# amzn/pecos

Hardware: AMD Instinct MI355X
Metric: XLinear queries/sec @ beam=10 top-k=10; P@1 vs reference; 1/2/4/8 GPU (higher is better)
Workload: dtype f32; 1 GPU; amazon-670k synthetic x1.0: N=490000 D=135000 L=670091 tree=[2, 32, 512, 8192, 670091] nnz/row=75.4 beam=10 topk=10 pp=l3-hinge bias=1.0; parallelism=query-shard x1

## Files before the change

pecos_amd/csrc/xrl_abi.cpp:

```cpp
#include "../../include/xrl_abi.h"

#include <algorithm>
#include <cfloat>
#include <chrono>
#include <cmath>
#include <cstdio>
#include <cstring>
#include <functional>
#include <condition_variable>
#include <memory>
#include <mutex>
#include <atomic>
#include <thread>
#include <unordered_map>

#include "xrl_predict.h"
#include "xrl_tfidf.h"

using namespace xrl;

namespace {
thread_local std::string g_err;
thread_local bool g_has_err = false;
thread_local int g_device = 0;
// ... 1265 lines not shown
    uint32_t n = 0;
    guarded([&] {
        Model& m = *as_model(model);
        resolve_profile(m);
        n = (uint32_t)m.profile.size();
        for (uint32_t i = 0; i < n && i < cap && out; ++i) {
            std::memset(&out[i], 0, sizeof(out[i]));
            std::strncpy(out[i].name, m.profile[i].name.c_str(), sizeof(out[i].name) - 1);
            out[i].layer = m.profile[i].layer; out[i].launches = m.profile[i].launches;
            out[i].ms = m.profile[i].ms;
        }
    });
    return n;
}

uint32_t xrl_debug_split_chunk(const uint64_t* cum, uint32_t n, uint64_t limit) {
    uint32_t v = 0;
    guarded([&] { if (!cum) fail("null cum"); v = split_chunk(cum, n, limit); });
    return v;
}

uint64_t xrl_debug_layout_rows(const uint32_t* rptr, uint32_t nrows, int align, uint32_t* ext_out) {
    uint64_t v = 0;
    guarded([&] { if (!rptr) fail("null rptr"); v = layout_tile_rows(rptr, nrows, align != 0, ext_out); });
    return v;
}

static void set_option_one(Model& m, const char* key, int64_t value) {
    if (!std::strcmp(key, "k1_group")) m.k1_group = (int)value;
    else if (!std::strcmp(key, "max_batch_rows")) m.max_batch_rows = value;
    else if (!std::strcmp(key, "sort_min_tiles")) m.sort_min_tiles = (int)value;
    else if (!std::strcmp(key, "sort_rest")) m.sort_rest = (int)value;
    else if (!std::strcmp(key, "prune_mid")) m.prune_mid = (int)value;
    else if (!std::strcmp(key, "tile_rows")) m.tile_rows = (int)value;
    else if (!std::strcmp(key, "k2_big_min_k")) m.k2_big_min_k = (int)value;
    else if (!std::strcmp(key, "qsort")) m.qsort = (int)value;
    else if (!std::strcmp(key, "qsort_min_parents")) m.qsort_min_parents = (int)value;
    else if (!std::strcmp(key, "qsort_min_rows")) m.qsort_min_rows = (int)value;
    else if (!std::strcmp(key, "presence")) m.presence = (int)value;
    else if (!std::strcmp(key, "adaptive")) { m.adaptive = (int)value; for (auto& u : m.fb_unstaged) u = 0; for (auto& u : m.fb_probing) u = 0; }
    else if (!std::strcmp(key, "host_pipeline")) m.host_pipeline = (int)value;
    else if (!std::strcmp(key, "host_batch_mb")) m.host_batch_mb = (int)value;
    else if (!std::strcmp(key, "sort_rest_min")) m.sort_rest_min = (int)value;
    else if (!std::strcmp(key, "reserve_rows")) {
        if (value < 0 || value > 0x7FFFFFFF) fail("reserve_rows: expected 0 .. 2^31-1");
        std::lock_guard<std::mutex> g(m.mu);
        use_device(m.device);
        if (!m.ws) m.ws = std::make_unique<Workspace>();
        reserve_outputs(m, (uint32_t)value, effective_topk(m, 0));
    }
    else if (!std::strcmp(key, "host_register")) m.host_register = (int)value;
    else if (!std::strcmp(key, "k1q_fuse")) m.k1q_fuse = (int)value;
    else if (!std::strcmp(key, "k1g_first")) m.k1g_first = (int)value;
    else if (!std::strcmp(key, "k1g_min_items")) m.k1g_min_items = (int)value;
    else if (!std::strcmp(key, "dense_layers")) m.dense_layers = (int)value;
    else if (!std::strcmp(key, "overlap_min_rows")) m.overlap_min_rows = (int)value;
    else if (!std::strcmp(key, "prune")) m.prune = (int)value;
    else if (!std::strcmp(key, "k1g_variant")) m.k1g_variant = (int)value;
    else if (!std::strcmp(key, "k1_wpb")) m.k1_wpb = (int)value;
    else if (!std::strcmp(key, "k1_lds_pad")) m.k1_lds_pad = (int)value;
    else if (!std::strcmp(key, "k1_ablate")) m.k1_ablate = (int)value;
    else fail(std::string("unknown option ") + key);
}


int xrl_set_option(void* model, const char* key, int64_t value) {
    int rc = -1;
    guarded([&] {
        Model& m = *as_model(model);
        if (!key) fail("null key");
        if (!std::strcmp(key, "devices")) {
            if (value < 1 || value > 64) fail("devices: expected 1..64");
            if (m.src_kind < 0 && value > 1) fail("devices: only models loaded from a folder can be replicated");
            std::lock_guard<std::mutex> g(m.mu);
            int ndev = 0;
            XRL_HIP(hipGetDeviceCount(&ndev));
            m.replicas.clear();
            for (int64_t i = 1; i < value; ++i) {
                const int dev = (m.device + (int)i) % std::max(1, ndev);
                use_device(dev);
                std::unique_ptr<Model> r = m.src_kind == 0 ? load_model_from_disk(m.src_path, m.weight_matrix_type) : load_mmap_model_from_disk(m.src_path);
                r->device = dev;
                r->k1_group = m.k1_group; r->max_batch_rows = m.max_batch_rows; r->sort_min_tiles = m.sort_min_tiles; r->sort_rest = m.sort_rest; r->sort_rest_min = m.sort_rest_min; r->prune_mid = m.prune_mid; r->tile_rows = m.tile_rows; r->k2_big_min_k = m.k2_big_min_k; r->qsort = m.qsort; r->qsort_min_parents = m.qsort_min_parents; r->qsort_min_rows = m.qsort_min_rows; r->presence = m.presence; r->adaptive = m.adaptive; r->host_pipeline = m.host_pipeline; r->host_batch_mb = m.host_batch_mb; r->host_register = m.host_register;
                r->k1q_fuse = m.k1q_fuse; r->k1g_min_items = m.k1g_min_items; r->k1g_first = m.k1g_first; r->dense_layers = m.dense_layers;
                r->overlap_min_rows = m.overlap_min_rows; r->prune = m.prune;
                r->k1g_variant = m.k1g_variant; r->k1_wpb = m.k1_wpb; r->k1_lds_pad = m.k1_lds_pad; r->k1_ablate = m.k1_ablate;
                m.replicas.push_back(std::move(r));
            }
            use_device(m.device);
        } else {
            set_option_one(m, key, value);
            for (auto& r : m.replicas) set_option_one(*r, key, value);
        }
        rc = 0;
    });
    return rc;
}

void xrl_debug_k1_phases(unsigned long long* out8, int reset) { guarded([&] { k1_phase_read(out8, reset != 0); }); }

uint32_t xrl_layer_info(void* model, uint32_t layer, uint64_t* out, uint32_t cap) {
    uint32_t n = 0;
    guarded([&] {
        Model& m = *as_model(model);
        if (layer >= m.layers.size()) fail("xrl_layer_info: layer out of range");
        const Layer& L = *m.layers[layer];
        const uint64_t rec[12] = {
            (uint64_t)(L.dev.bucket ? 1 : (L.dev.bitmap64 ? 2 : 0)), L.bk_levels, (uint64_t)(L.dev.wd ? 1 : 0), 1ull << L.dev.d_gp_log2,
            L.dev.d_ld, L.n_tiles, L.nnz, L.dense_bytes, L.w_rows, L.n_children, L.max_tile_cols, L.device_bytes};
        n = 12;
        for (uint32_t i = 0; i < n && i < cap && out; ++i) out[i] = rec[i];
    });
    return n;
}

uint64_t xrl_model_device_bytes(void* model) {
// ... 271 lines not shown
```

pecos_amd/csrc/xrl_device.h:

```cpp
#pragma once
#include <hip/hip_runtime.h>

#include <cfloat>
#include <cmath>

#include "xrl_model.h"

namespace xrl {

__device__ __forceinline__ void wave_sync_lds() {
    __builtin_amdgcn_fence(__ATOMIC_SEQ_CST, "wavefront");
    __builtin_amdgcn_wave_barrier();
}

__device__ __forceinline__ bool prune_guard_ok(uint32_t xmax_bits, uint32_t n_feat, float wmax) {
    if (xmax_bits >= 0x7F800000u) return false;
    const float b = fmaxf(__uint_as_float(xmax_bits), 1.0f) * wmax * (float)(n_feat + 2u);
    return b < 1.0e37f;
}

__device__ __forceinline__ float ref_expf(float x) { return (float)exp((double)x); }

__device__ __forceinline__ double hinge_pow4(float zf, int p) {
    const double z = (double)zf;
// ... 95 lines not shown
template <int NS>
__device__ __forceinline__ uint32_t wave_topk_extract(uint32_t (&kx)[NS], const uint32_t (&sbits)[NS], const uint32_t (&payload)[NS],
                                                      uint32_t k, int lane, uint32_t& o_rank, uint32_t& o_sbits, uint32_t& o_payload) {
    uint32_t osb = 0, opl = 0, i = 0;
    for (; i < k; ++i) {
        uint32_t m = kx[0];
#pragma unroll
        for (int r = 1; r < NS; ++r) m = max(m, kx[r]);
        const uint32_t mx = wave_max_u32(m);
        if (mx == 0u) break;
        bool found = false;
#pragma unroll
        for (int r = 0; r < NS; ++r) {
            if (!found) {
                const unsigned long long b = __ballot(kx[r] == mx);
                if (b != 0ull) {
                    const int wl = __builtin_ctzll(b);
                    const int sb = __builtin_amdgcn_readlane((int)sbits[r], wl), pl = __builtin_amdgcn_readlane((int)payload[r], wl);
                    const bool dst = (uint32_t)lane == i;
                    osb = dst ? (uint32_t)sb : osb;
                    opl = dst ? (uint32_t)pl : opl;
                    kx[r] = lane == wl ? 0u : kx[r];
                    found = true;
                }
            }
        }
    }
    o_rank = (uint32_t)lane; o_sbits = osb; o_payload = opl;
    return i;
}
constexpr uint32_t kTopkExtractMaxK = 20;

template <int NS>
__device__ __forceinline__ uint32_t wave_topk(uint32_t (&key)[NS], const uint32_t (&sbits)[NS], const uint32_t (&payload)[NS],
                                              uint32_t k, uint2* sc, int lane, uint32_t& o_rank, uint32_t& o_sbits, uint32_t& o_payload) {
    if (k <= kTopkExtractMaxK) return wave_topk_extract<NS>(key, sbits, payload, k, lane, o_rank, o_sbits, o_payload);
    o_rank = 0; o_sbits = 0; o_payload = 0;
    const uint32_t n_valid = wave_count_ge<NS>(key, 1u);
    const uint32_t kk = min(k, n_valid);
    if (kk == 0) return 0;
    uint32_t lo = 1u, hi = 0xFFFFFFFFu;
    bool exact = false;
    if (NS >= 4) {
        uint32_t m[1] = {key[0]};
#pragma unroll
        for (int r = 1; r < NS; ++r) m[0] = max(m[0], key[r]);
        uint32_t mx = m[0];
#pragma unroll
        for (int d = 1; d < 64; d <<= 1) mx = max(mx, (uint32_t)__shfl_xor((int)mx, d, 64));
        hi = __builtin_amdgcn_readfirstlane(mx);
        bool e1;
        lo = wave_bisect_kth<1>(m, kk, 0u, hi, e1);
        if (lo == 0u) lo = 1u;
    }
    const uint32_t T = wave_bisect_kth<NS>(key, kk, lo, hi, exact);
    uint32_t need_eq = 0;
    if (!exact) need_eq = kk - (T == 0xFFFFFFFFu ? 0u : wave_count_ge<NS>(key, T + 1u));
    uint32_t base = 0, eq_seen = 0;
#pragma unroll
    for (int r = 0; r < NS; ++r) {
        const bool above = exact ? key[r] >= T : key[r] > T;
        const bool eq = !exact && key[r] == T;
        const unsigned long long meq = __ballot(eq);
        const bool sel = above || (eq && eq_seen + lanes_below(meq) < need_eq);
        const unsigned long long msel = __ballot(sel);
        if (sel) sc[base + lanes_below(msel)] = make_uint2(sbits[r], payload[r]);
// ... 17 lines not shown
```

pecos_amd/csrc/xrl_k1t.hip:

```cpp
#include <hip/hip_runtime.h>

#include <cfloat>
#include <cmath>

#include "xrl_device.h"
#include "xrl_kernels.h"
#include "xrl_items.h"

namespace xrl {

#define XRL_LAUNCH_CHECK() XRL_HIP(hipGetLastError())

namespace {

__device__ __forceinline__ uint32_t xcd_remap_t(uint32_t b, uint32_t nb) {
    const uint32_t xcd = b & 7u, q = nb >> 3, r = nb & 7u;
    const uint32_t base = (xcd < r) ? xcd * (q + 1u) : r * (q + 1u) + (xcd - r) * q;
    return base + (b >> 3);
}

struct K1TArgs {
    LayerDev L;
    QueriesDev X;
    const ItemDesc* items;
    const uint32_t* n_items;
    float* cand;
    uint64_t n_slots;
    int pp_kind, pp_p, first_layer, bias_first;
    uint32_t n_vblocks;
    uint32_t* fb_out;
    uint32_t wt_bytes;
};

template <int NR> struct RowVec;
template <> struct RowVec<1> { float v[1]; };
template <> struct alignas(8) RowVec<2> { float v[2]; };
template <> struct RowVec<3> { float v[3]; };
template <> struct alignas(16) RowVec<4> { float v[4]; };

typedef uint32_t u32x2 __attribute__((ext_vector_type(2)));
typedef uint32_t u32x3 __attribute__((ext_vector_type(3)));
typedef uint32_t u32x4 __attribute__((ext_vector_type(4)));
template <int NR> __device__ __forceinline__ RowVec<NR> row_load_buf(__amdgpu_buffer_rsrc_t rs, uint32_t voff);
template <> __device__ __forceinline__ RowVec<1> row_load_buf<1>(__amdgpu_buffer_rsrc_t rs, uint32_t voff) { return __builtin_bit_cast(RowVec<1>, __builtin_amdgcn_raw_buffer_load_b32(rs, (int)voff, 0, 0)); }
template <> __device__ __forceinline__ RowVec<2> row_load_buf<2>(__amdgpu_buffer_rsrc_t rs, uint32_t voff) { return __builtin_bit_cast(RowVec<2>, __builtin_amdgcn_raw_buffer_load_b64(rs, (int)voff, 0, 0)); }
template <> __device__ __forceinline__ RowVec<3> row_load_buf<3>(__amdgpu_buffer_rsrc_t rs, uint32_t voff) {
    const auto t = __builtin_amdgcn_raw_buffer_load_b96(rs, (int)voff, 0, 0);
    RowVec<3> r; r.v[0] = __uint_as_float(t[0]); r.v[1] = __uint_as_float(t[1]); r.v[2] = __uint_as_float(t[2]); return r;
}
template <> __device__ __forceinline__ RowVec<4> row_load_buf<4>(__amdgpu_buffer_rsrc_t rs, uint32_t voff) { return __builtin_bit_cast(RowVec<4>, __builtin_amdgcn_raw_buffer_load_b128(rs, (int)voff, 0, 0)); }

template <int G, int NR, int PPC, int LK, bool BUF>
__global__ void __launch_bounds__(256) __attribute__((amdgpu_waves_per_eu(5, 8))) k1t_kernel(K1TArgs a) {
    constexpr int W = 64 / G, H = 64, U = (G >= 16) ? 64 / G : 8, UNR = 8, STRIDE = G * NR;
    __shared__ uint2 hq_all[4 * W * (H + UNR)];
    const uint32_t wave = threadIdx.x >> 6;
    const uint32_t vblock = blockIdx.x * 4u + wave;
    if (vblock >= a.n_vblocks) return;
    const int lane = threadIdx.x & 63;
    const int grp = lane / G, lig = lane % G;
    uint2* __restrict__ my_hq = hq_all + ((size_t)wave * W + grp) * (H + UNR);

    ItemDesc it = make_item(0u, kNoTile, 0u, 0.f, 0, 0u);
    if (a.n_items) {
        const uint32_t n = *a.n_items, nb = (n + W - 1) / W;
        if (a.fb_out && vblock == 0 && lane == 0) *a.fb_out = n;
        if (vblock >= nb) return;
        { const uint64_t slot = (uint64_t)xcd_remap_t(vblock, nb) * W + grp; if (slot < n) it = a.items[slot]; }
    } else {
        const uint64_t slot = (uint64_t)vblock * W + grp;
        if (slot < a.n_slots) it = a.items[slot];
    }
    const bool active = it.tile != kNoTile;
    TileDesc td{};
    uint64_t xe = 0, cur = 0, wbase = 0;
    if (active) {
        td = a.L.tiles[it.tile];
        wbase = a.L.wt_base[it.tile];
        cur = it.x_begin; xe = it.x_begin + it.x_len;
    }
    const char* __restrict__ wrow = reinterpret_cast<const char*>(a.L.wt + (BUF ? 0ull : wbase) + (uint32_t)(NR * lig));
    const uint32_t tbase = BUF ? (uint32_t)(wbase * 4ull) : 0u;
    const uint32_t lane_off = (uint32_t)(NR * lig * 4);
    const __amdgpu_buffer_rsrc_t wrs = __builtin_amdgcn_make_buffer_rsrc(const_cast<float*>(a.L.wt), 0, (int)(BUF ? a.wt_bytes : 0u), 0x00020000);
    const uint32_t pad_off = tbase + td.nrows * (uint32_t)(STRIDE * 4);
    float acc[NR];
    {
        const float* __restrict__ bp = a.L.bias_prod + td.col_begin;
#pragma unroll
        for (int k = 0; k < NR; ++k) {
            const uint32_t c = (uint32_t)(NR * lig + k);
            acc[k] = (a.bias_first && a.L.has_bias && c < td.ncols) ? bp[c] : 0.0f;
        }
    }
    const uint32_t* __restrict__ xi = a.X.col_idx;
    const float* __restrict__ xv = a.X.val;
    const BmWord* __restrict__ bm = a.L.bitmap + (LK != 0 ? 0ull : (uint64_t)(active ? it.tile : 0u) * a.L.nwords);
    const BmWord64* __restrict__ bm64 = a.L.bitmap64 + (LK != 2 ? 0ull : (uint64_t)(active ? it.tile : 0u) * a.L.nwords64);
    const unsigned long long below = (1ull << lig) - 1ull;
    const uint64_t xlast = xe > cur ? xe - 1 : 0;
    uint32_t nh = 0;
    bool nonfin = false;

    auto drain = [&](auto exact_tag) {
        constexpr bool EX = decltype(exact_tag)::value;
        wave_sync_lds();
// ... 60 lines not shown
#pragma unroll
                for (int u = 0; u < U; ++u) {
                    const bool inr = f[u] != 0xFFFFFFFFu;
                    const BmWord64 wi = bm64[inr ? (f[u] >> 6) : 0u];
                    const uint32_t b = f[u] & 63u;
                    const unsigned long long bits = ((unsigned long long)wi.hi << 32) | wi.lo;
                    hit[u] = inr && ((bits >> b) & 1ull);
                    off[u] = tbase + (wi.rank + (uint32_t)__popcll(bits & ((1ull << b) - 1ull))) * (uint32_t)(STRIDE * 4);
                }
            }
            uint32_t done = skip;
            bool stopped = false;
#pragma unroll
            for (int u = 0; u < U; ++u) {
                const unsigned long long m = __ballot(hit[u]);
                const unsigned long long gm = (G == 64) ? m : ((m >> (grp * G)) & ((1ull << G) - 1ull));
                const uint32_t cnt = (uint32_t)__popcll(gm);
                if ((uint32_t)u >= done && !stopped) {
                    if (nh + cnt <= (uint32_t)H) {
                        if (hit[u]) my_hq[nh + (uint32_t)__popcll(gm & below)] = make_uint2(__float_as_uint(v[u]), off[u]);
                        nh += cnt; done = u + 1;
                    } else {
                        stopped = true;
                    }
                }
            }
            if (done == (uint32_t)U) { if (cur < xe) cur += (uint64_t)U * G; skip = 0; }
            else { skip = done; overflow = true; }
        }
        if (__any(overflow)) drain_any();
    }
    drain_any();

    if (!active) return;
    float* __restrict__ out = a.cand + it.out_off;
    const float* __restrict__ bp = a.L.bias_prod + td.col_begin;
    const bool add_bias = a.L.has_bias != 0 && !a.bias_first;
#pragma unroll
    for (int k = 0; k < NR; ++k) {
        const uint32_t c = (uint32_t)(NR * lig + k);
        if (c < td.ncols) {
            float s = acc[k];
            if (add_bias) s = __fadd_rn(s, bp[c]);
            float v = pp_transform<PPC>(a.pp_kind, a.pp_p, s);
            if (!a.first_layer) v = pp_combine(a.pp_kind, v, it.pscore);
            out[c] = v;
        }
    }
}

__global__ void __launch_bounds__(256)
tile_rows_kernel(const TileDesc* __restrict__ tiles, const uint32_t* __restrict__ row_ext, const Entry* __restrict__ entries,
                 const uint64_t* __restrict__ wt_base, uint32_t stride, uint32_t* __restrict__ wt) {
    const TileDesc td = tiles[blockIdx.x];
    uint32_t* __restrict__ dst = wt + wt_base[blockIdx.x];
    const uint32_t* __restrict__ ext = row_ext + td.rowptr_base;
    const Entry* __restrict__ ent = entries + td.ent_base;
    const uint32_t sub = threadIdx.x >> 5, l = threadIdx.x & 31u;
    for (uint32_t r = sub; r < td.nrows; r += 8u) {
        const uint32_t e = ext[r], start = e & 0x1FFFFFFu, len = (e >> 25) + 1u;
        for (uint32_t i = l; i < len; i += 32u) {
            const Entry x = ent[start + i];
            const uint32_t b = __float_as_uint(x.val);
            dst[(uint64_t)r * stride + x.col] = b == kMissing ? 0u : b;
        }
    }
}

}

void k1t_shape(uint32_t max_tile_cols, int& g, int& nr) {
    g = max_tile_cols <= 8 ? 8 : max_tile_cols <= 16 ? 16 : 32;
    nr = (int)((max_tile_cols + (uint32_t)g - 1) / (uint32_t)g);
    if (nr < 1) nr = 1;
}

void launch_tile_rows(const LayerDev& L, uint64_t total_floats, uint32_t* wt, hipStream_t s) {
    XRL_HIP(hipMemsetD32Async(reinterpret_cast<hipDeviceptr_t>(wt), (int)kMissing, total_floats, s));
    if (L.n_tiles) {
        hipLaunchKernelGGL(tile_rows_kernel, dim3(L.n_tiles), dim3(256), 0, s, L.tiles, L.row_ext, L.entries, L.wt_base, L.wt_stride, wt);
        XRL_LAUNCH_CHECK();
    }
}

bool k1t_serves(const LayerDev& L, const QueriesDev& X) { return L.wt != nullptr && !X.dense && (L.bitmap || L.bitmap64) && !L.bucket; }

void launch_k1t(const LayerDev& L, const LayerPlan& P, const QueriesDev& X, const void* items, const uint32_t* n_items, float* cand, hipStream_t s) {
    if (P.nrows == 0) return;
    K1TArgs a;
    a.L = L; a.X = X; a.items = static_cast<const ItemDesc*>(items); a.n_items = n_items; a.cand = cand;
    a.n_slots = (uint64_t)P.nrows * P.beam_in * L.max_tiles_per_parent;
    a.pp_kind = P.pp.kind; a.pp_p = P.pp.p; a.first_layer = P.first_layer; a.bias_first = P.bias_first;
    a.fb_out = (n_items && P.fb_host && P.layer >= 0 && P.layer < 16) ? P.fb_host + 32 + P.layer : nullptr;
    int g, nr;
    k1t_shape(L.max_tile_cols, g, nr);
    if ((uint32_t)(g * nr) != L.wt_stride || nr > 4) fail("k1t: the layer's tile rows were laid out for another shape");
    const uint64_t vblocks = (a.n_slots + (uint64_t)(64 / g) - 1) / (uint64_t)(64 / g);
    if (vblocks > 0x7FFFFFFFull) fail("k1t: grid too large; lower max_batch_rows");
    a.n_vblocks = (uint32_t)vblocks;
    const dim3 grid((uint32_t)((vblocks + 3) / 4)), block(256);
    const int ppc = pp_class(P.pp);
    const int lk = L.bitmap64 ? 2 : 0;
    const bool buf = L.wt_bytes != 0 && L.wt_bytes < 0xFFFFFF00ull;
    a.wt_bytes = buf ? (uint32_t)L.wt_bytes : 0u;
#define XRL_K1T_B(GG, NN, BB) do { \
        if (ppc) { if (lk) hipLaunchKernelGGL((k1t_kernel<GG, NN, 1, 2, BB>), grid, block, 0, s, a); else hipLaunchKernelGGL((k1t_kernel<GG, NN, 1, 0, BB>), grid, block, 0, s, a); } \
        else     { if (lk) hipLaunchKernelGGL((k1t_kernel<GG, NN, 0, 2, BB>), grid, block, 0, s, a); else hipLaunchKernelGGL((k1t_kernel<GG, NN, 0, 0, BB>), grid, block, 0, s, a); } } while (0)
#define XRL_K1T(GG, NN) do { if (buf) XRL_K1T_B(GG, NN, true); else XRL_K1T_B(GG, NN, false); } while (0)
    if (g == 8) XRL_K1T(8, 1);
    else if (g == 16) XRL_K1T(16, 1);
    else if (nr == 1) XRL_K1T(32, 1);
    else if (nr == 2) XRL_K1T(32, 2);
    else if (nr == 3) XRL_K1T(32, 3);
    else XRL_K1T(32, 4);
#undef XRL_K1T
#undef XRL_K1T_B
    XRL_LAUNCH_CHECK();
}

}
```

pecos_amd/csrc/xrl_kernels.h:

```cpp
#pragma once
#include "xrl_model.h"

namespace xrl {

struct QueriesDev {
    const uint64_t* row_ptr;
    const uint32_t* col_idx;
    const float* val;
    uint32_t rows, cols;
    int dense;
    uint64_t nnz;
};

struct BeamDev {
    uint32_t* idx;
    float* val;
    uint32_t* cnt;
    uint32_t stride;
};

struct K1Tune { int wpb = 1, lds_pad = 0, ablate = 0, k1g_variant = 0, pres_mode = 1, tile_rows = 1, k2_big_min_k = 0; };

struct LayerPlan {
    uint32_t row0, nrows;
// ... 31 lines not shown
void launch_k2_topk(const LayerDev& L, const LayerPlan& P, BeamDev prev, const uint32_t* cand_off,
                    const uint32_t* ncand, const float* cand, uint32_t* out_idx, float* out_val,
                    uint32_t* out_cnt, uint32_t out_stride, hipStream_t s,
                    uint32_t rank_limit = 0 , uint32_t limited_cands = 0 ,
                    uint32_t* done = nullptr , const uint32_t* skip_done = nullptr ,
                    const uint32_t* xok = nullptr );
constexpr int kStatsPerLayer = 8;
void launch_stats(const LayerDev& L, const LayerPlan& P, const QueriesDev& X, BeamDev prev, const uint32_t* ncand, const void* items,
                  double* out8, hipStream_t s, uint64_t item_slots = 0 );
void launch_k3_inner_products(const uint64_t* x_ptr, const uint32_t* x_idx, const float* x_val, int x_dense,
                              const uint64_t* w_ptr, const uint32_t* w_idx, const float* w_val, int w_dense,
                              uint32_t dim, uint64_t len, const uint32_t* rows, const uint32_t* cols,
                              float* out, hipStream_t s);

unsigned long long* k1_phase_buffer();
void k1_phase_read(unsigned long long out[8], bool reset);
void launch_k4_selected(const uint64_t* col_ptr, const uint32_t* row_idx, const float* val, uint32_t w_rows, float bias,
                        const QueriesDev& X, const uint32_t* pair_q, const uint32_t* node, const uint32_t* ppos,
                        const uint64_t* prev_off, const float* prev_val, float* out_val, uint64_t n_pairs,
                        const PostProc& pp, int first_layer, hipStream_t s);
uint32_t k1g_cols(const LayerDev& L);
void launch_k1g(const LayerDev& L, const LayerPlan& P, const QueriesDev& X, const void* items_sorted, const uint32_t* start,
                uint32_t* blk_start, const uint32_t* x_ok, float* cand, hipStream_t s);
void launch_xguard(const QueriesDev& X, uint32_t row0, uint32_t nrows, float wmax, uint32_t* ok, hipStream_t s);
void launch_k1c_csc(const LayerDev& L, const uint64_t* col_ptr, const uint32_t* row_idx, const float* val, const LayerPlan& P,
                    const QueriesDev& X, BeamDev prev, const uint32_t* cand_off, const uint32_t* ncand, float* cand, hipStream_t s);
void launch_concat_csr(const uint64_t* in_ptr, const uint32_t* in_idx, const float* in_val, const float* emb, uint32_t rows,
                       uint32_t sparse_cols, uint32_t dense_cols, int normalize_emb, uint64_t* out_ptr, uint32_t* out_idx, float* out_val, hipStream_t s);
void launch_tfidf_weight(const uint64_t* row_ptr, const uint32_t* col_idx, const float* count, const float* idf, uint32_t rows, uint32_t cols,
                         int binary, int sublinear_tf, int norm_p, float* out, hipStream_t s,
                         uint32_t seg_stride = 1, uint32_t seg_off = 0, uint32_t* err = nullptr);
int k1_auto_group(const LayerDev& L, const Layer& host, int dense);
bool k1t_serves(const LayerDev& L, const QueriesDev& X);
void launch_k1t(const LayerDev& L, const LayerPlan& P, const QueriesDev& X, const void* items, const uint32_t* n_items, float* cand, hipStream_t s);
uint32_t k1q_regs(const LayerDev& L, uint32_t beam_in, uint32_t k, bool dense_x);
void launch_k1q(const LayerDev* const* Ls, const LayerPlan* Ps, int n, const QueriesDev& X, BeamDev prev, uint32_t* out_idx, float* out_val,
                uint32_t* out_cnt, uint32_t out_stride, hipStream_t s, float prune_wmax, uint32_t* out_xok = nullptr,
                const uint32_t* qperm = nullptr );
size_t k2_max_k();
void launch_k2_topk_big(const LayerDev& L, const LayerPlan& P, BeamDev prev, const uint32_t* cand_off, const uint32_t* ncand, const float* cand,
                        uint32_t* out_idx, float* out_val, uint32_t* out_cnt, uint32_t out_stride, hipStream_t s);

}
```

pecos_amd/csrc/xrl_model.h:

```cpp
#pragma once
#include <memory>
#include <mutex>
#include <string>
#include <vector>

#include "xrl_common.h"
#include "xrl_io.h"

namespace xrl {

constexpr uint32_t kMaxTileCols = 128;
constexpr uint32_t kNoBias = 0xFFFFFFFFu;
constexpr uint32_t kMissing = 0x80000000u;

enum PPKind : int { PP_NOOP = 0, PP_SIGMOID = 1, PP_LOG_SIGMOID = 2, PP_LP_HINGE = 3, PP_LOG_LP_HINGE = 4 };
struct PostProc { int kind = PP_NOOP; int p = 0; };
PostProc parse_post_processor(const char* name);

struct TileDesc {
    uint32_t col_begin;
    uint32_t ncols;
    uint32_t nrows;
    uint32_t bias_slot;
    uint64_t rowptr_base;
// ... 101 lines not shown
    hipStream_t d2h_stream = nullptr;
    std::vector<hipEvent_t> d2h_events;
    int host_register = 0;
    int host_batch_mb = 12;
    int host_pipeline = 1;
    std::vector<hipEvent_t> events;
    struct HostLanes { hipEvent_t done[2] = {nullptr, nullptr}; hipStream_t strm[2] = {nullptr, nullptr}; hipEvent_t join = nullptr; } host_lanes;
    std::mutex mu;
    std::unique_ptr<Workspace> ws;
    int k1_group = 0;
    int k1_wpb = 1, k1_lds_pad = 0, k1_ablate = 0;
    int k1g_variant = 0;
    int64_t max_batch_rows = 0;
    int overlap_min_rows = 0;
    int prune = 1;
    int k2_big_min_k = 0;
    int tile_rows = 1;
    int dense_layers = 1;
    bool csc_route = false;
    int k1q_fuse = 3;
    int k1g_first = 0;
    int k1g_min_items = 16;
    static constexpr int kFbLayers = 16;
    uint32_t* fb_host = nullptr;
    DevBuf fb_dev;
    DevBuf d_wd01;
    uint32_t fb_seen[kFbLayers] = {0}, fb_second[kFbLayers] = {0};
    uint64_t fb_tile_slots[kFbLayers] = {0};
    uint32_t fb_unstaged_calls[kFbLayers] = {0};
    uint8_t fb_unstaged[kFbLayers] = {0};
    uint8_t fb_probing[kFbLayers] = {0};
    int adaptive = 1;
    int presence = 1;
    int prune_mid = 1;
    int sort_rest = 1;
    int sort_rest_min = 32768;
    int qsort = 1;
    int qsort_min_parents = 64, qsort_min_rows = 131072;
    int sort_min_tiles = 0;
    std::string src_path; int src_kind = -1;
    std::vector<std::unique_ptr<Model>> replicas;
    bool profiling = false;
    std::vector<ProfileSlot> profile;
    std::vector<PendingEvent> pending;
    Model();
    ~Model();
    uint64_t device_bytes() const;
};

uint32_t split_chunk(const uint64_t* cum, uint32_t n, uint64_t limit);
uint64_t layout_tile_rows(const uint32_t* rptr, uint32_t nrows, bool align, uint32_t* ext);

std::unique_ptr<Layer> compile_layer(const HostCsc& W, const HostCsc& C, float bias, uint32_t only_topk,
                                     const std::string& post_processor,
                                     const std::vector<uint32_t>* perm_inv_override = nullptr, uint32_t orig_rows = 0,
                                     bool structure_only = false);
std::unique_ptr<Model> load_model_from_disk(const std::string& path, int weight_matrix_type);
void finalize_model(Model& m);
std::unique_ptr<Model> load_mmap_model_from_disk(const std::string& path);
void compile_mmap_model(const std::string& npz_path, const std::string& mmap_path);
void ensure_device_csc(Layer& L);
void k1t_shape(uint32_t max_tile_cols, int& g, int& nr);
void launch_tile_rows(const LayerDev& L, uint64_t total_floats, uint32_t* wt, hipStream_t s);
void launch_merge01(const uint32_t* wd0, uint64_t ld0, uint32_t k0, const uint32_t* wd1, uint64_t ld1, uint32_t c1, uint32_t rows, uint32_t* out, hipStream_t s);
void launch_presence(const uint32_t* wd, uint64_t ld, uint32_t rows, uint32_t gp_log2, uint32_t n_tiles, uint32_t pres_words, uint32_t* pres, hipStream_t s);
void launch_densify(const uint64_t* col_ptr, const uint32_t* row_idx, const float* val, const uint32_t* src_col,
// ... 4 lines not shown
```

pecos_amd/csrc/xrl_predict.cpp:

```cpp
#include "xrl_predict.h"

#include <algorithm>
#include <cstdio>
#include <cstdlib>

namespace xrl {

namespace {
size_t profile_slot(Model& m, const char* name, uint32_t layer) {
    for (size_t i = 0; i < m.profile.size(); ++i)
        if (m.profile[i].layer == layer && m.profile[i].name == name) return i;
    m.profile.push_back(ProfileSlot{name, layer});
    return m.profile.size() - 1;
}
}

static uint32_t k1g_first_slots(const Layer& L, uint32_t beam_in, int forced = 0) {
    if (forced > 0) return (uint32_t)std::max<int64_t>(1, std::min<int64_t>(beam_in > 1 ? (int64_t)beam_in - 1 : 1, forced));
    return (uint32_t)std::max<uint64_t>(1, std::min<uint64_t>(beam_in > 1 ? beam_in - 1 : 1, 64 / std::max<uint64_t>(1, L.cand_bound(1))));
}

uint32_t effective_topk(const Model& m, uint32_t only_topk) {
    return only_topk ? only_topk : m.layers.back()->only_topk;
}
// ... 284 lines not shown
                    continue;
                }
                uint32_t *qi, *qc; float* qv; uint32_t qs;
                beam_out(l1, qi, qv, qc, qs);
                timed(launch_name(l, l1).c_str(), (uint32_t)l, [&] { launch_k1q(Ls, Ps, (int)(l1 - l + 1), X, prev, qi, qv, qc, qs, S, prune_wmax, xok_out); });
                l = l1;
                continue;
            }
            int g = m.k1_group > 0 ? m.k1_group : k1_auto_group(L.dev, L, X.dense);
            int mode = layer_mode(l, nrows);
            const bool fb_unstaged = l < (size_t)Model::kFbLayers && unst[l];
            if (fb_unstaged && mode == 0 && sorts_rest(l)) mode = 1;
            bool pruned = m.prune && !fb_unstaged && !P.implicit_root && !P.first_layer && P.pp.kind != PP_NOOP && beam_in[l] > 1 && k2_wave_path(P);
            uint32_t J = 1;
            if (o.stats_out) {
                const bool dense_x = X.dense != 0 || m.dense_layers >= 2;
                if (mode == 3) J = k1g_first_slots(L, beam_in[l], m.k1g_first);
                else if (m.dense_layers && k1q_regs(L.dev, beam_in[l], k[l], dense_x) != 0) {
                    if (k1q_regs(L.dev, beam_in[l], k[l], dense_x) <= 1) pruned = false;
                    else J = std::max<uint32_t>(1, (64u >> L.dev.d_gp_log2) / std::max<uint32_t>(1, L.dev.d_max_tiles));
                }
                if (J >= beam_in[l]) pruned = false;
            } else if (mode != 0) pruned = false;
            if (pruned) {
                uint32_t stage_end[3]; int n_stage = 0;
                stage_end[n_stage++] = J;
                if (m.prune_mid != 0 && beam_in[l] >= 16u && !o.stats_out) stage_end[n_stage++] = std::min<uint32_t>(beam_in[l] - 1u, J + 4u);
                stage_end[n_stage++] = beam_in[l];
                const uint64_t slots_b = (uint64_t)nrows * (beam_in[l] - J) * L.max_tiles_per_parent;
                lw.prune_done.reserve((size_t)nb * 4); lw.prune_cnt.reserve(256);
                lw.items_sorted.reserve(slots_max * k0_item_bytes());
                need_x_ok();
                LayerPlan PA = P; PA.beam_in = J;
                timed("k0_prolongate", (uint32_t)l, [&] { launch_k0_prolongate(L.dev, P, X, prev, lw.cand_off.as<uint32_t>(), lw.ncand.as<uint32_t>(), lw.items.p, S, J); });
                if (lanes == 2 && k1_done) XRL_HIP(hipStreamWaitEvent(S, k1_done, 0));
                timed(X.dense ? "k1_dense" : "k1_sparse", (uint32_t)l, [&] { launch_k1(L.dev, PA, X, lw.items.p, nullptr, lw.cand.as<float>(), g, S); });
                timed("k2_topk", (uint32_t)l, [&] { launch_k2_topk(L.dev, P, prev, lw.cand_off.as<uint32_t>(), lw.ncand.as<uint32_t>(), lw.cand.as<float>(), oi, ov, oc, os, S,
                                                                   J, (uint32_t)L.cand_bound(J), lw.prune_done.as<uint32_t>(), nullptr, lw.x_ok.as<uint32_t>()); });
                if (o.stats_out) XRL_HIP(hipMemsetAsync(lw.items_sorted.p, 0xFF, slots_b * k0_item_bytes(), S));
                bool srt = sorts_rest(l);
                if (srt && P.fb_host && l < (size_t)Model::kFbLayers && m.sort_rest_min > 0) {
                    const uint32_t seen = static_cast<volatile uint32_t*>(m.fb_host)[2 * Model::kFbLayers + l];
                    const uint64_t need = std::max<uint64_t>((uint64_t)m.sort_rest_min, 32ull * L.n_tiles);
                    if (seen != 0xFFFFFFFFu && (uint64_t)seen < need) srt = false;
                }
                if (P.fb_host && l < (size_t)Model::kFbLayers) m.fb_tile_slots[l] = (uint64_t)nrows * (beam_in[l] - stage_end[n_stage - 2]) * L.max_tiles_per_parent;
                for (int st = 1; st < n_stage; ++st) {
                    const uint32_t r0 = stage_end[st - 1], r1 = stage_end[st];
                    const bool last = st == n_stage - 1;
                    const uint64_t slots_s = (uint64_t)nrows * (r1 - r0) * L.max_tiles_per_parent;
                    LayerPlan PB = P; PB.beam_in = r1 - r0;
                    PB.tune.wpb = 4;
                    const char* sfx = last ? "_rest" : "_mid";
                    timed(last ? "k0b_remaining" : "k0b_remaining_mid", (uint32_t)l, [&] { launch_k0b_remaining(L.dev, P, X, prev, lw.cand_off.as<uint32_t>(), lw.prune_done.as<uint32_t>(), r0,
                                                                                                                 srt ? lw.items.p : lw.items_sorted.p, lw.prune_cnt.as<uint32_t>(), S, r1); });
                    if (srt) timed((std::string("k1_sort_items") + sfx).c_str(), (uint32_t)l, [&] { launch_sort_items(L.dev, slots_s, lw.items.p, lw.items_sorted.p, lw.sort_hist.as<uint32_t>(),
                                                                                                                      lw.sort_start.as<uint32_t>(), S, lw.prune_cnt.as<uint32_t>()); });
                    timed((std::string(X.dense ? "k1_dense" : "k1_sparse") + sfx).c_str(), (uint32_t)l, [&] {
                        launch_k1(L.dev, PB, X, lw.items_sorted.p, srt ? lw.sort_start.as<uint32_t>() + L.n_tiles : lw.prune_cnt.as<uint32_t>(), lw.cand.as<float>(), g, S); });
                    if (lanes == 2 && last) { k1_done = next_event(); XRL_HIP(hipEventRecord(k1_done, S)); }
                    if (last) timed("k2_topk_rest", (uint32_t)l, [&] { launch_k2_topk(L.dev, P, prev, lw.cand_off.as<uint32_t>(), lw.ncand.as<uint32_t>(), lw.cand.as<float>(), oi, ov, oc, os, S,
                                                                                      0, 0, nullptr, lw.prune_done.as<uint32_t>()); });
                    else timed("k2_topk_mid", (uint32_t)l, [&] { launch_k2_topk(L.dev, P, prev, lw.cand_off.as<uint32_t>(), lw.ncand.as<uint32_t>(), lw.cand.as<float>(), oi, ov, oc, os, S,
                                                                                 r1, (uint32_t)L.cand_bound(r1), lw.prune_done.as<uint32_t>(), lw.prune_done.as<uint32_t>(), lw.x_ok.as<uint32_t>()); });
                    if (o.stats_out && last) {
                        launch_stats(L.dev, P, X, prev, lw.ncand.as<uint32_t>(), lw.items.p, ws.stats.as<double>() + kStatsPerLayer * l, S, (uint64_t)nrows * J * L.max_tiles_per_parent);
                        launch_stats(L.dev, PB, X, prev, nullptr, lw.items_sorted.p, ws.stats.as<double>() + kStatsPerLayer * l, S, slots_b);
                    }
                }
                continue;
            }
// ... 48 lines not shown
```

Before: 92.10 million queries/s.

## Fuse leaf-layer item derivation and top-k selection into k1t kernel epilogue

Adds a selecting epilogue to the tiled k1t scoring kernel. In pruned layers with a single first-stage parent it ranks each query's top-k with a half-wavefront extract, decides the bound-pruning done flag, and computes candidate offsets in place. Optionally it also derives work items directly from the previous beam, so the k0_prolongate and k2_topk launches are skipped. This removes two kernel launches and the round trip of candidate scores through global memory, at the cost of more register pressure and extra template instances. It is enabled by default through a new leaf_fuse option.

```diff
diff --git a/pecos_amd/csrc/xrl_abi.cpp b/pecos_amd/csrc/xrl_abi.cpp
--- a/pecos_amd/csrc/xrl_abi.cpp
+++ b/pecos_amd/csrc/xrl_abi.cpp
@@ -1321,6 +1321,7 @@
     else if (!std::strcmp(key, "sort_min_tiles")) m.sort_min_tiles = (int)value;
     else if (!std::strcmp(key, "sort_rest")) m.sort_rest = (int)value;
     else if (!std::strcmp(key, "prune_mid")) m.prune_mid = (int)value;
+    else if (!std::strcmp(key, "leaf_fuse")) m.leaf_fuse = (int)value;
     else if (!std::strcmp(key, "tile_rows")) m.tile_rows = (int)value;
     else if (!std::strcmp(key, "k2_big_min_k")) m.k2_big_min_k = (int)value;
     else if (!std::strcmp(key, "qsort")) m.qsort = (int)value;
@@ -1370,7 +1371,7 @@
                 use_device(dev);
                 std::unique_ptr<Model> r = m.src_kind == 0 ? load_model_from_disk(m.src_path, m.weight_matrix_type) : load_mmap_model_from_disk(m.src_path);
                 r->device = dev;
-                r->k1_group = m.k1_group; r->max_batch_rows = m.max_batch_rows; r->sort_min_tiles = m.sort_min_tiles; r->sort_rest = m.sort_rest; r->sort_rest_min = m.sort_rest_min; r->prune_mid = m.prune_mid; r->tile_rows = m.tile_rows; r->k2_big_min_k = m.k2_big_min_k; r->qsort = m.qsort; r->qsort_min_parents = m.qsort_min_parents; r->qsort_min_rows = m.qsort_min_rows; r->presence = m.presence; r->adaptive = m.adaptive; r->host_pipeline = m.host_pipeline; r->host_batch_mb = m.host_batch_mb; r->host_register = m.host_register;
+                r->k1_group = m.k1_group; r->max_batch_rows = m.max_batch_rows; r->sort_min_tiles = m.sort_min_tiles; r->sort_rest = m.sort_rest; r->sort_rest_min = m.sort_rest_min; r->prune_mid = m.prune_mid; r->leaf_fuse = m.leaf_fuse; r->tile_rows = m.tile_rows; r->k2_big_min_k = m.k2_big_min_k; r->qsort = m.qsort; r->qsort_min_parents = m.qsort_min_parents; r->qsort_min_rows = m.qsort_min_rows; r->presence = m.presence; r->adaptive = m.adaptive; r->host_pipeline = m.host_pipeline; r->host_batch_mb = m.host_batch_mb; r->host_register = m.host_register;
                 r->k1q_fuse = m.k1q_fuse; r->k1g_min_items = m.k1g_min_items; r->k1g_first = m.k1g_first; r->dense_layers = m.dense_layers;
                 r->overlap_min_rows = m.overlap_min_rows; r->prune = m.prune;
                 r->k1g_variant = m.k1g_variant; r->k1_wpb = m.k1_wpb; r->k1_lds_pad = m.k1_lds_pad; r->k1_ablate = m.k1_ablate;
diff --git a/pecos_amd/csrc/xrl_device.h b/pecos_amd/csrc/xrl_device.h
--- a/pecos_amd/csrc/xrl_device.h
+++ b/pecos_amd/csrc/xrl_device.h
@@ -151,6 +151,49 @@
 constexpr uint32_t kTopkExtractMaxK = 20;
 
 template <int NS>
+__device__ __forceinline__ void halfwave_topk_extract(uint32_t (&kx)[NS], const uint32_t (&sbits)[NS], uint32_t k, int lane,
+                                                      uint32_t& o_sbits, uint32_t& o_pos, uint32_t& kk_lo, uint32_t& kk_hi) {
+    const bool hi = lane >= 32;
+    const uint32_t lig = (uint32_t)lane & 31u;
+    uint32_t osb = 0, ops = 0, nlo = 0, nhi = 0;
+    for (uint32_t i = 0; i < k; ++i) {
+        uint32_t x = kx[0];
+#pragma unroll
+        for (int r = 1; r < NS; ++r) x = max(x, kx[r]);
+        x = max(x, (uint32_t)__builtin_amdgcn_update_dpp(0, (int)x, 0xB1, 0xF, 0xF, true));
+        x = max(x, (uint32_t)__builtin_amdgcn_update_dpp(0, (int)x, 0x4E, 0xF, 0xF, true));
+        x = max(x, (uint32_t)__builtin_amdgcn_update_dpp(0, (int)x, 0x141, 0xF, 0xF, true));
+        x = max(x, (uint32_t)__builtin_amdgcn_update_dpp(0, (int)x, 0x140, 0xF, 0xF, true));
+        const uint32_t mlo = max((uint32_t)__builtin_amdgcn_readlane((int)x, 0), (uint32_t)__builtin_amdgcn_readlane((int)x, 16));
+        const uint32_t mhi = max((uint32_t)__builtin_amdgcn_readlane((int)x, 32), (uint32_t)__builtin_amdgcn_readlane((int)x, 48));
+        if ((mlo | mhi) == 0u) break;
+        const uint32_t mx = hi ? mhi : mlo;
+        bool hit = false;
+        uint32_t msb = 0, mr = 0;
+#pragma unroll
+        for (int r = NS - 1; r >= 0; --r) {
+            const bool e = kx[r] == mx;
+            msb = e ? sbits[r] : msb; mr = e ? (uint32_t)r : mr; hit = hit || e;
+        }
+        hit = hit && mx != 0u;
+        const unsigned long long b = __ballot(hit);
+        const uint32_t blo = (uint32_t)b, bhi = (uint32_t)(b >> 32);
+        const int wlo = blo ? __builtin_ctz(blo) : 0, whi = 32 + (bhi ? __builtin_ctz(bhi) : 0);
+        const uint32_t mps = (uint32_t)NS * lig + mr;
+        const uint32_t sb_lo = (uint32_t)__builtin_amdgcn_readlane((int)msb, wlo), ps_lo = (uint32_t)__builtin_amdgcn_readlane((int)mps, wlo);
+        const uint32_t sb_hi = (uint32_t)__builtin_amdgcn_readlane((int)msb, whi), ps_hi = (uint32_t)__builtin_amdgcn_readlane((int)mps, whi);
+        const bool dst = lig == i;
+        osb = dst ? (hi ? sb_hi : sb_lo) : osb;
+        ops = dst ? (hi ? ps_hi : ps_lo) : ops;
+        const bool win = hit && lane == (hi ? whi : wlo);
+#pragma unroll
+        for (int r = 0; r < NS; ++r) kx[r] = (win && mr == (uint32_t)r) ? 0u : kx[r];
+        nlo += mlo != 0u ? 1u : 0u; nhi += mhi != 0u ? 1u : 0u;
+    }
+    o_sbits = osb; o_pos = ops; kk_lo = nlo; kk_hi = nhi;
+}
+
+template <int NS>
 __device__ __forceinline__ uint32_t wave_topk(uint32_t (&key)[NS], const uint32_t (&sbits)[NS], const uint32_t (&payload)[NS],
                                               uint32_t k, uint2* sc, int lane, uint32_t& o_rank, uint32_t& o_sbits, uint32_t& o_payload) {
     if (k <= kTopkExtractMaxK) return wave_topk_extract<NS>(key, sbits, payload, k, lane, o_rank, o_sbits, o_payload);
diff --git a/pecos_amd/csrc/xrl_k1t.hip b/pecos_amd/csrc/xrl_k1t.hip
--- a/pecos_amd/csrc/xrl_k1t.hip
+++ b/pecos_amd/csrc/xrl_k1t.hip
@@ -30,6 +30,13 @@
     uint32_t n_vblocks;
     uint32_t* fb_out;
     uint32_t wt_bytes;
+    const uint32_t* p_cnt; const float* p_val; uint32_t p_stride, beam_in;
+    const uint32_t* xok; const uint32_t* perm_inv;
+    uint32_t* out_idx; float* out_val; uint32_t* out_cnt; uint32_t* done;
+    uint32_t out_stride, k;
+    int mult;
+    const uint32_t* p_idx; const uint64_t* x_row_ptr;
+    uint32_t cand_stride; uint32_t* cand_off; uint32_t* ncand;
 };
 
 template <int NR> struct RowVec;
@@ -50,7 +57,7 @@
 }
 template <> __device__ __forceinline__ RowVec<4> row_load_buf<4>(__amdgpu_buffer_rsrc_t rs, uint32_t voff) { return __builtin_bit_cast(RowVec<4>, __builtin_amdgcn_raw_buffer_load_b128(rs, (int)voff, 0, 0)); }
 
-template <int G, int NR, int PPC, int LK, bool BUF>
+template <int G, int NR, int PPC, int LK, bool BUF, bool SEL>
 __global__ void __launch_bounds__(256) __attribute__((amdgpu_waves_per_eu(5, 8))) k1t_kernel(K1TArgs a) {
     constexpr int W = 64 / G, H = 64, U = (G >= 16) ? 64 / G : 8, UNR = 8, STRIDE = G * NR;
     __shared__ uint2 hq_all[4 * W * (H + UNR)];
@@ -61,6 +68,15 @@
     const int grp = lane / G, lig = lane % G;
     uint2* __restrict__ my_hq = hq_all + ((size_t)wave * W + grp) * (H + UNR);
 
+    auto derive_item = [&](uint64_t q) {
+        const uint32_t cnt = min(a.p_cnt[q], a.beam_in);
+        const uint32_t parent = cnt ? a.p_idx[q * a.p_stride] : 0u;
+        const float ps = a.p_val[q * a.p_stride];
+        const uint64_t xb = a.x_row_ptr[q];
+        const uint32_t xl = (uint32_t)(a.x_row_ptr[q + 1] - xb);
+        const uint32_t t0 = a.L.ptile[parent], t1 = a.L.ptile[parent + 1];
+        return make_item((uint32_t)q, (cnt && t1 > t0) ? t0 : kNoTile, (uint32_t)q * a.cand_stride, ps, xb, xl);
+    };
     ItemDesc it = make_item(0u, kNoTile, 0u, 0.f, 0, 0u);
     if (a.n_items) {
         const uint32_t n = *a.n_items, nb = (n + W - 1) / W;
@@ -69,9 +85,9 @@
         { const uint64_t slot = (uint64_t)xcd_remap_t(vblock, nb) * W + grp; if (slot < n) it = a.items[slot]; }
     } else {
         const uint64_t slot = (uint64_t)vblock * W + grp;
-        if (slot < a.n_slots) it = a.items[slot];
-    }
-    const bool active = it.tile != kNoTile;
+        if (slot < a.n_slots) it = (SEL && !a.items) ? derive_item(slot) : a.items[slot];
+    }
+    bool active = it.tile != kNoTile;
     TileDesc td{};
     uint64_t xe = 0, cur = 0, wbase = 0;
     if (active) {
@@ -198,6 +214,76 @@
     }
     drain_any();
 
+    if constexpr (SEL) {
+        static_assert(G == 32, "the selecting epilogue ranks one item per half-wavefront");
+        int lane_e = lane;
+        asm volatile("" : "+v"(lane_e));
+        const int grp = lane_e >> 5, lig = lane_e & 31;
+        const uint64_t slot = (uint64_t)vblock * W + grp;
+        const bool qv = slot < a.n_slots;
+        const uint64_t q = qv ? slot : 0;
+        if constexpr (NR == 4) {
+            it = a.items ? a.items[q] : derive_item(q);
+            active = qv && it.tile != kNoTile;
+            td = a.L.tiles[active ? it.tile : 0u];
+        }
+        const uint32_t pc = a.p_cnt[q], xok = a.xok[q];
+        const float ps_next = a.p_val[q * a.p_stride + 1u];
+        const float* __restrict__ bp = a.L.bias_prod + td.col_begin;
+        const bool add_bias = a.L.has_bias != 0 && !a.bias_first;
+        uint32_t key[NR], sb[NR];
+#pragma unroll
+        for (int k = 0; k < NR; ++k) {
+            const uint32_t c = (uint32_t)(NR * lig + k);
+            key[k] = 0u; sb[k] = 0u;
+            if (active && c < td.ncols) {
+                float s = acc[k];
+                if (add_bias) s = __fadd_rn(s, bp[c]);
+                float v = pp_transform<PPC>(a.pp_kind, a.pp_p, s);
+                if (!a.first_layer) v = pp_combine(a.pp_kind, v, it.pscore);
+                sb[k] = __float_as_uint(v); key[k] = score_key(v);
+            }
+        }
+        const bool limited = min(pc, a.beam_in) > 1u;
+        const uint32_t thr = score_key(a.mult ? fmaxf(ps_next, 0.0f) : ps_next);
+        uint32_t c_lo = 0, c_hi = 0;
+#pragma unroll
+        for (int k = 0; k < NR; ++k) {
+            const unsigned long long b = __ballot(key[k] >= thr);
+            c_lo += (uint32_t)__popc((uint32_t)b); c_hi += (uint32_t)__popc((uint32_t)(b >> 32));
+        }
+        const bool d = !limited || (xok != 0u && ps_next == ps_next && (grp ? c_hi : c_lo) >= a.k);
+        if (!a.items && __any(qv && !d)) {
+            const uint32_t cnt = min(pc, a.beam_in);
+            const bool mine = qv && !d && (uint32_t)lig < cnt;
+            uint32_t wd = 0;
+            if (mine) { const uint32_t pj = a.p_idx[q * a.p_stride + (uint32_t)lig]; wd = a.L.chunk_col[pj + 1] - a.L.chunk_col[pj]; }
+            uint32_t incl = wd;
+#pragma unroll
+            for (int s = 1; s < 32; s <<= 1) { const uint32_t y = (uint32_t)__shfl_up((int)incl, s, 32); if (lig >= s) incl += y; }
+            const uint32_t total = (uint32_t)__shfl((int)incl, 31, 32);
+            if (mine) a.cand_off[q * a.beam_in + (uint32_t)lig] = incl - wd;
+            if (qv && !d && lig == 0) a.ncand[q] = total;
+        }
+        if (active && !d) {
+            float* __restrict__ out = a.cand + it.out_off;
+#pragma unroll
+            for (int k = 0; k < NR; ++k) { const uint32_t c = (uint32_t)(NR * lig + k); if (c < td.ncols) out[c] = __uint_as_float(sb[k]); }
+        }
+        uint32_t osb, ops, kk_lo, kk_hi;
+        halfwave_topk_extract<NR>(key, sb, a.k, lane_e, osb, ops, kk_lo, kk_hi);
+        const uint32_t kk = grp ? kk_hi : kk_lo;
+        if (qv) {
+            if ((uint32_t)lig < kk) {
+                uint32_t child = td.col_begin + ops;
+                if (a.perm_inv) child = a.perm_inv[child];
+                a.out_idx[q * a.out_stride + (uint32_t)lig] = child;
+                a.out_val[q * a.out_stride + (uint32_t)lig] = __uint_as_float(osb);
+            }
+            if (lig == 0) { a.out_cnt[q] = kk; a.done[q] = d ? 1u : 0u; }
+        }
+        return;
+    }
     if (!active) return;
     float* __restrict__ out = a.cand + it.out_off;
     const float* __restrict__ bp = a.L.bias_prod + td.col_begin;
@@ -251,11 +337,19 @@
 
 bool k1t_serves(const LayerDev& L, const QueriesDev& X) { return L.wt != nullptr && !X.dense && (L.bitmap || L.bitmap64) && !L.bucket; }
 
-void launch_k1t(const LayerDev& L, const LayerPlan& P, const QueriesDev& X, const void* items, const uint32_t* n_items, float* cand, hipStream_t s) {
+bool k1t_selects(const LayerDev& L, const LayerPlan& P, const QueriesDev& X) {
+    int g, nr;
+    k1t_shape(L.max_tile_cols, g, nr);
+    return k1t_serves(L, X) && P.tune.tile_rows >= 1 && P.tune.ablate == 0 && L.max_tiles_per_parent == 1 && g == 32 && nr <= 4 &&
+           P.k >= 1 && P.k <= kTopkExtractMaxK && P.beam_in >= 2 && !P.implicit_root && !P.first_layer && k2_wave_path(P);
+}
+
+void launch_k1t(const LayerDev& L, const LayerPlan& P, const QueriesDev& X, const void* items, const uint32_t* n_items, float* cand, hipStream_t s,
+                const K1TSelect* sel) {
     if (P.nrows == 0) return;
-    K1TArgs a;
+    K1TArgs a{};
     a.L = L; a.X = X; a.items = static_cast<const ItemDesc*>(items); a.n_items = n_items; a.cand = cand;
-    a.n_slots = (uint64_t)P.nrows * P.beam_in * L.max_tiles_per_parent;
+    a.n_slots = sel ? (uint64_t)P.nrows : (uint64_t)P.nrows * P.beam_in * L.max_tiles_per_parent;
     a.pp_kind = P.pp.kind; a.pp_p = P.pp.p; a.first_layer = P.first_layer; a.bias_first = P.bias_first;
     a.fb_out = (n_items && P.fb_host && P.layer >= 0 && P.layer < 16) ? P.fb_host + 32 + P.layer : nullptr;
     int g, nr;
@@ -264,23 +358,39 @@
     const uint64_t vblocks = (a.n_slots + (uint64_t)(64 / g) - 1) / (uint64_t)(64 / g);
     if (vblocks > 0x7FFFFFFFull) fail("k1t: grid too large; lower max_batch_rows");
     a.n_vblocks = (uint32_t)vblocks;
-    const dim3 grid((uint32_t)((vblocks + 3) / 4)), block(256);
     const int ppc = pp_class(P.pp);
     const int lk = L.bitmap64 ? 2 : 0;
     const bool buf = L.wt_bytes != 0 && L.wt_bytes < 0xFFFFFF00ull;
     a.wt_bytes = buf ? (uint32_t)L.wt_bytes : 0u;
-#define XRL_K1T_B(GG, NN, BB) do { \
-        if (ppc) { if (lk) hipLaunchKernelGGL((k1t_kernel<GG, NN, 1, 2, BB>), grid, block, 0, s, a); else hipLaunchKernelGGL((k1t_kernel<GG, NN, 1, 0, BB>), grid, block, 0, s, a); } \
-        else     { if (lk) hipLaunchKernelGGL((k1t_kernel<GG, NN, 0, 2, BB>), grid, block, 0, s, a); else hipLaunchKernelGGL((k1t_kernel<GG, NN, 0, 0, BB>), grid, block, 0, s, a); } } while (0)
-#define XRL_K1T(GG, NN) do { if (buf) XRL_K1T_B(GG, NN, true); else XRL_K1T_B(GG, NN, false); } while (0)
+    if (sel) {
+        if (n_items || !k1t_selects(L, P, X)) fail("k1t: the selecting epilogue does not serve this launch");
+        if (!sel->done || !sel->xok) fail("k1t: bound pruning needs the done and the per-query guard flags");
+        a.p_cnt = sel->prev.cnt; a.p_val = sel->prev.val; a.p_stride = sel->prev.stride; a.beam_in = P.beam_in;
+        a.xok = sel->xok; a.perm_inv = L.perm_inv;
+        a.out_idx = sel->out_idx; a.out_val = sel->out_val; a.out_cnt = sel->out_cnt; a.done = sel->done;
+        a.out_stride = sel->out_stride; a.k = P.k;
+        a.mult = (P.pp.kind == PP_SIGMOID || P.pp.kind == PP_LP_HINGE) ? 1 : 0;
+        if (!items) {
+            if (!sel->cand_off || !sel->ncand || P.beam_in > 32u) fail("k1t: the launch cannot derive its items");
+            if ((uint64_t)P.nrows * P.cand_stride > 0xFFFFFFFFull) fail("k1t: candidate buffer exceeds 2^32 floats; lower max_batch_rows");
+            a.p_idx = sel->prev.idx; a.x_row_ptr = X.row_ptr + P.row0; a.cand_stride = P.cand_stride; a.cand_off = sel->cand_off; a.ncand = sel->ncand;
+        }
+    }
+    const dim3 grid((a.n_vblocks + 3u) / 4u), block(256);
+#define XRL_K1T_L(GG, NN, BB, SS) do { \
+        if (ppc) { if (lk) hipLaunchKernelGGL((k1t_kernel<GG, NN, 1, 2, BB, SS>), grid, block, 0, s, a); else hipLaunchKernelGGL((k1t_kernel<GG, NN, 1, 0, BB, SS>), grid, block, 0, s, a); } \
+        else     { if (lk) hipLaunchKernelGGL((k1t_kernel<GG, NN, 0, 2, BB, SS>), grid, block, 0, s, a); else hipLaunchKernelGGL((k1t_kernel<GG, NN, 0, 0, BB, SS>), grid, block, 0, s, a); } } while (0)
+#define XRL_K1T(GG, NN) do { if (buf) XRL_K1T_L(GG, NN, true, false); else XRL_K1T_L(GG, NN, false, false); } while (0)
+#define XRL_K1T_S(NN) do { if (sel) { if (buf) XRL_K1T_L(32, NN, true, true); else XRL_K1T_L(32, NN, false, true); } else XRL_K1T(32, NN); } while (0)
     if (g == 8) XRL_K1T(8, 1);
     else if (g == 16) XRL_K1T(16, 1);
-    else if (nr == 1) XRL_K1T(32, 1);
-    else if (nr == 2) XRL_K1T(32, 2);
-    else if (nr == 3) XRL_K1T(32, 3);
-    else XRL_K1T(32, 4);
+    else if (nr == 1) XRL_K1T_S(1);
+    else if (nr == 2) XRL_K1T_S(2);
+    else if (nr == 3) XRL_K1T_S(3);
+    else XRL_K1T_S(4);
+#undef XRL_K1T_S
 #undef XRL_K1T
-#undef XRL_K1T_B
+#undef XRL_K1T_L
     XRL_LAUNCH_CHECK();
 }
 
diff --git a/pecos_amd/csrc/xrl_kernels.h b/pecos_amd/csrc/xrl_kernels.h
--- a/pecos_amd/csrc/xrl_kernels.h
+++ b/pecos_amd/csrc/xrl_kernels.h
@@ -87,7 +87,10 @@
                          uint32_t seg_stride = 1, uint32_t seg_off = 0, uint32_t* err = nullptr);
 int k1_auto_group(const LayerDev& L, const Layer& host, int dense);
 bool k1t_serves(const LayerDev& L, const QueriesDev& X);
-void launch_k1t(const LayerDev& L, const LayerPlan& P, const QueriesDev& X, const void* items, const uint32_t* n_items, float* cand, hipStream_t s);
+struct K1TSelect { BeamDev prev; const uint32_t* xok; uint32_t* out_idx; float* out_val; uint32_t* out_cnt; uint32_t out_stride; uint32_t* done; uint32_t* cand_off; uint32_t* ncand; };
+bool k1t_selects(const LayerDev& L, const LayerPlan& P, const QueriesDev& X);
+void launch_k1t(const LayerDev& L, const LayerPlan& P, const QueriesDev& X, const void* items, const uint32_t* n_items, float* cand, hipStream_t s,
+                const K1TSelect* sel = nullptr);
 uint32_t k1q_regs(const LayerDev& L, uint32_t beam_in, uint32_t k, bool dense_x);
 void launch_k1q(const LayerDev* const* Ls, const LayerPlan* Ps, int n, const QueriesDev& X, BeamDev prev, uint32_t* out_idx, float* out_val,
                 uint32_t* out_cnt, uint32_t out_stride, hipStream_t s, float prune_wmax, uint32_t* out_xok = nullptr,
diff --git a/pecos_amd/csrc/xrl_model.h b/pecos_amd/csrc/xrl_model.h
--- a/pecos_amd/csrc/xrl_model.h
+++ b/pecos_amd/csrc/xrl_model.h
@@ -157,6 +157,7 @@
     uint8_t fb_probing[kFbLayers] = {0};
     int adaptive = 1;
     int presence = 1;
+    int leaf_fuse = 1;
     int prune_mid = 1;
     int sort_rest = 1;
     int sort_rest_min = 32768;
diff --git a/pecos_amd/csrc/xrl_predict.cpp b/pecos_amd/csrc/xrl_predict.cpp
--- a/pecos_amd/csrc/xrl_predict.cpp
+++ b/pecos_amd/csrc/xrl_predict.cpp
@@ -340,11 +340,18 @@
                 lw.items_sorted.reserve(slots_max * k0_item_bytes());
                 need_x_ok();
                 LayerPlan PA = P; PA.beam_in = J;
-                timed("k0_prolongate", (uint32_t)l, [&] { launch_k0_prolongate(L.dev, P, X, prev, lw.cand_off.as<uint32_t>(), lw.ncand.as<uint32_t>(), lw.items.p, S, J); });
+                const bool fuse = m.leaf_fuse != 0 && J == 1 && !o.stats_out && k1t_selects(L.dev, P, X);
+                const bool fuse_k0 = fuse && m.leaf_fuse != 2 && beam_in[l] <= 32u;
+                if (!fuse_k0) timed("k0_prolongate", (uint32_t)l, [&] { launch_k0_prolongate(L.dev, P, X, prev, lw.cand_off.as<uint32_t>(), lw.ncand.as<uint32_t>(), lw.items.p, S, J); });
                 if (lanes == 2 && k1_done) XRL_HIP(hipStreamWaitEvent(S, k1_done, 0));
+                if (fuse) {
+                    const K1TSelect sel{prev, lw.x_ok.as<uint32_t>(), oi, ov, oc, os, lw.prune_done.as<uint32_t>(), lw.cand_off.as<uint32_t>(), lw.ncand.as<uint32_t>()};
+                    timed("k1_sparse", (uint32_t)l, [&] { launch_k1t(L.dev, P, X, fuse_k0 ? nullptr : lw.items.p, nullptr, lw.cand.as<float>(), S, &sel); });
+                } else {
                 timed(X.dense ? "k1_dense" : "k1_sparse", (uint32_t)l, [&] { launch_k1(L.dev, PA, X, lw.items.p, nullptr, lw.cand.as<float>(), g, S); });
                 timed("k2_topk", (uint32_t)l, [&] { launch_k2_topk(L.dev, P, prev, lw.cand_off.as<uint32_t>(), lw.ncand.as<uint32_t>(), lw.cand.as<float>(), oi, ov, oc, os, S,
                                                                    J, (uint32_t)L.cand_bound(J), lw.prune_done.as<uint32_t>(), nullptr, lw.x_ok.as<uint32_t>()); });
+                }
                 if (o.stats_out) XRL_HIP(hipMemsetAsync(lw.items_sorted.p, 0xFF, slots_b * k0_item_bytes(), S));
                 bool srt = sorts_rest(l);
                 if (srt && P.fb_host && l < (size_t)Model::kFbLayers && m.sort_rest_min > 0) {
```

Result: faster. 97.79 million queries/s, median of 6 (+6.2%).
